# qiaozhijian/gf-orb-slam2

Measured on AMD Instinct MI355X. Metric: frames/sec ORB extract+match, 752x480 @2000 kp, higher is better.
Workload: dtype u8; 1 GPU; configs[2]: stereo 752x480 pair, 2000 features/image, extract L+R + stereo Hamming match; frame=one camera image (a stereo pair = 2 frames + 1 association), width=752, height=480, nfeatures=2000, levels=8, contexts_per_gpu=2, contexts_chained_after_stage=1, priming_steps=48, distinct_input_batches=4

## Files before the change

gf-orb-slam2_amd/csrc/gfo_api.hip:

```cpp
#include "gfo_internal.h"

#include <math.h>
#include <stdarg.h>
#include <stdio.h>
#include <stdlib.h>
#include <string.h>

static std::string g_create_err;
#include <algorithm>
#include <mutex>
#include <vector>
#include <atomic>
static std::mutex g_ctx_mu;
static std::vector<gfo_ctx*> g_ctx_live;
static std::atomic<int> g_contexts_created{0}, g_arenas_planned{0};

int gfo_fail(gfo_ctx* c, int code, const char* fmt, ...)
{
    char buf[512];
    va_list ap;
    va_start(ap, fmt);
    vsnprintf(buf, sizeof buf, fmt, ap);
    va_end(ap);
    if (c) c->err = buf;
// ... 95 lines not shown
    c->quota[n - 1] = c->prm.nfeatures - sum > 0 ? c->prm.nfeatures - sum : 0;
}

static void free_arena(gfo_ctx* c)
{
    void* ptrs[] = {c->d_geom, c->d_input, c->d_pyr, c->d_blur, c->d_cand, c->d_cand_cnt, c->d_node_of, c->d_sel,
                    c->d_sel_cnt, c->d_kp, c->d_desc, c->d_kp_cnt, c->d_flags, c->d_xofs, c->d_xcoef, c->d_yofs, c->d_band, c->d_cell_tab, c->d_qt_scratch,
                    c->d_ycoef, c->st.u_right, c->st.depth, c->st.best_dist, c->st.best_idx, c->st.nmatched, c->st.counted,
                    c->d_scale, c->d_inv_scale, c->d_kp_un, c->st_sort.sx, c->st_sort.sy, c->st_sort.soi, c->st_sort.sdesc, c->st_sort.row_start, c->st_sort.lorder, c->st_sort.lrow_start};
    for (void* p : ptrs)
        if (p) (void)hipFree(p);
    c->d_geom = nullptr; c->d_input = c->d_pyr = c->d_blur = nullptr; c->d_cand = nullptr; c->d_cand_cnt = nullptr;
    c->d_node_of = nullptr; c->d_sel = nullptr; c->d_sel_cnt = nullptr; c->d_kp = nullptr; c->d_desc = nullptr;
    c->d_kp_cnt = nullptr; c->d_flags = nullptr; c->d_xofs = nullptr; c->d_xcoef = nullptr; c->d_yofs = nullptr; c->d_band = nullptr; c->d_cell_tab = nullptr; c->d_od_tab = nullptr; c->od_pairs = 0; c->d_qt_scratch = nullptr;
    c->d_ycoef = nullptr; c->st = GfoStereoDev{}; c->d_scale = nullptr; c->d_inv_scale = nullptr; c->d_kp_un = nullptr; c->st_sort = GfoStereoSort{}; c->st_rows_cap = 0;
    c->planned = false;
    c->have_batch = c->have_pyramid = c->have_stereo = false;
    c->plan_gen++;
    if (c->graph_exec) {
        (void)hipGraphExecDestroy(c->graph_exec);
        c->graph_exec = nullptr;
    }
}

static void resize_tables(int ssize, int dsize, int* ofs, short* coef, bool clamp_x)
{
    const double inv_scale = (double)dsize / ssize;
    const double scale = 1. / inv_scale;
    for (int d = 0; d < dsize; d++) {
        float f = (float)((d + 0.5) * scale - 0.5);
        int s = (int)floorf(f);
        f -= s;
        if (clamp_x) {
            if (s < 0) { f = 0; s = 0; }
            if (s >= ssize - 1) { f = 0; s = ssize - 1; }
        }
        ofs[d] = s;
        coef[2 * d] = (short)lrintf((1.f - f) * 2048.f);
        coef[2 * d + 1] = (short)lrintf(f * 2048.f);
    }
}

#if GFO_OCV_RESIZE == 1
static void resize_tables_float(int ssize, int dsize, int* ofs, int* frac_bits)
{
    const double scale = 1. / ((double)dsize / ssize);
    for (int d = 0; d < dsize; d++) {
        float f = (float)((d + 0.5) * scale - 0.5);
        int s = (int)floorf(f);
        f -= s;
        if (s < 0) { f = 0; s = 0; }
        if (s >= ssize - 1) { f = 0; s = ssize - 1; }
        ofs[d] = s;
        memcpy(&frac_bits[d], &f, 4);
    }
}
#endif

int gfo_plan(gfo_ctx* c, int w, int h, int batch)
{
    if (c->planned && c->g.w0 == w && c->g.h0 == h && batch <= c->cap_batch) return GFO_OK;
    if (w > 4000 || h > 4000) return fail(c, GFO_ERR_INVALID, "image %dx%d exceeds the 4000-px coordinate packing", w, h);
    const int keep_batch = c->planned && c->g.w0 == w && c->g.h0 == h ? c->cap_batch : 0;
    (void)hipStreamSynchronize(c->stream);
    free_arena(c);
    batch = batch > keep_batch ? batch : keep_batch;
    if (batch < c->prm.max_batch) batch = c->prm.max_batch;
    GfoGeom& g = c->g;
    memset(&g, 0, sizeof g);
    g.nlevels = c->prm.nlevels;
    g.w0 = w;
    g.h0 = h;
    g.ini_th = c->prm.ini_th_fast;
    g.min_th = c->prm.min_th_fast;
    long long pyr_off = 0, blur_off = 0, cand_off = 0;
    int cell_base = 0, tile_base = 0, blur_b = 0, sel_off = 0, xtab = 0, ytab = 0;
    int max_cw = 8, max_ch = 8;
    for (int l = 0; l < g.nlevels; l++) {
        GfoLevel& L = g.lv[l];
        const float s = c->inv_scale[l];
        L.w = (int)lrintf((float)w * s);
        L.h = (int)lrintf((float)h * s);
        if (L.w < 1 || L.h < 1) return fail(c, GFO_ERR_INVALID, "level %d of a %dx%d image is empty", l, w, h);
        L.pitch = (int)align_up(L.w, 64);
        L.plane_off = pyr_off;
        if (l > 0) pyr_off += align_up((long long)L.pitch * L.h, 256);
        L.blur_off = blur_off;
        blur_off += align_up((long long)L.pitch * L.h, 256);
        L.max_bx = L.w - GFO_EDGE + 3;
        L.max_by = L.h - GFO_EDGE + 3;
        const float width = (float)(L.max_bx - GFO_MIN_BORDER), height = (float)(L.max_by - GFO_MIN_BORDER);
        L.cell_base = cell_base;
        if (width >= (float)GFO_CELL_W && height >= (float)GFO_CELL_W) {
            L.ncols = (int)(width / GFO_CELL_W);
            L.nrows = (int)(height / GFO_CELL_W);
            L.wcell = (int)ceilf(width / L.ncols);
            L.hcell = (int)ceilf(height / L.nrows);
            cell_base += L.ncols * L.nrows;
            max_cw = L.wcell + 6 > max_cw ? L.wcell + 6 : max_cw;
            max_ch = L.hcell + 6 > max_ch ? L.hcell + 6 : max_ch;
            L.cand_cap = L.ncols * L.nrows * ((L.wcell + 1) / 2) * ((L.hcell + 1) / 2);
        } else {
            L.ncols = L.nrows = 0;
            L.wcell = L.hcell = 1;
            L.cand_cap = 0;
        }
        L.cand_off = cand_off;
        cand_off += align_up(L.cand_cap, 64);
        L.tiles_x = (L.w + 3) / 4;
        L.tiles_y = (L.h + GFO_BLUR_STRIP - 1) / GFO_BLUR_STRIP;
        {
            int nint = (L.w - 8) / 4;
            if (nint > L.tiles_x - 1) nint = L.tiles_x - 1;
            if (nint < 0) nint = 0;
            L.tile_base = tile_base;
            tile_base += (nint * L.tiles_y + 255) / 256;
            L.blur_base_b = blur_b;
            blur_b += ((L.tiles_x - nint) * L.tiles_y + 255) / 256;
        }
        L.quota = c->quota[l];
        int nini = 1;
        if (L.max_by - GFO_MIN_BORDER > 0) nini = (int)roundf(width / height);
        if (nini < 1) nini = 1;
        L.n_ini = nini;
        L.hx = width / nini;
        L.node_cap = (L.quota > 4 * nini ? L.quota : 4 * nini) + 8;
        L.sel_off = sel_off;
        L.sel_cap = L.node_cap;
        sel_off += L.sel_cap;
        L.scale = c->scale[l];
        L.patch_size = (int)(GFO_PATCH * c->scale[l]);
        L.xtab_off = xtab;
        L.ytab_off = ytab;
        if (l > 0) {
            xtab += (int)align_up(L.w + 3, 4) + 4;
            ytab += (int)align_up(L.h + 3, 4) + 4;
        }
        if (L.node_cap > 60000) return fail(c, GFO_ERR_INVALID, "level %d takes %d of the %d features: more than 60000 nodes per level are not supported", l, L.quota, c->prm.nfeatures);
    }
    if (max_cw - 6 > 64 || max_ch - 6 > 64)
        return fail(c, GFO_ERR_INVALID, "FAST cell %dx%d exceeds the per-wave plan", max_cw - 6, max_ch - 6);
    const int xtab_n = xtab, ytab_n = ytab;
    g.total_cells = cell_base;
    g.total_tiles = tile_base;
    g.blur_total_b = blur_b;
    g.total_sel_cap = sel_off;
    g.kp_stride = (int)align_up(sel_off, 4);
    g.fast_tile_pitch = max_cw <= 45 ? 48 : (max_cw <= 61 ? 64 : 80);
    g.fast_npx_max = (int)align_up((long long)(max_cw - 6) * (max_ch - 6), 8);
    {
        const int qcap_env = getenv("GFO_FAST_QCAP") ? atoi(getenv("GFO_FAST_QCAP")) : 0;
        const int qc = qcap_env >= 264 ? (qcap_env & ~7) : GFO_FAST_QCAP;
        g.fast_q_cap = g.fast_npx_max < qc ? g.fast_npx_max : qc;
    }
    g.fast_tile_rows = max_ch;
    g.fast_smap_pitch = g.fast_tile_pitch - 4;
    g.fast_smap_rows = (int)align_up((long long)(max_ch - 6 + 2) * g.fast_smap_pitch, 16) / g.fast_smap_pitch + 1;
    g.pyr_img_stride = align_up(pyr_off, 256);
    g.blur_img_stride = align_up(blur_off, 256);
    g.cand_img_stride = align_up(cand_off, 64);
    if (g.kp_stride > 65535) return fail(c, GFO_ERR_INVALID, "more than 65535 keypoints per image are not supported");

    std::vector<int> xtabv(2 * (size_t)(xtab_n > 0 ? xtab_n : 4)), ytabv(2 * (size_t)(ytab_n > 0 ? ytab_n : 4));
    for (int l = 1; l < g.nlevels; l++) {
        const int dw = g.lv[l].w, dh = g.lv[l].h;
        std::vector<int> ofs(dw > dh ? dw : dh);
        std::vector<short> coef(2 * ofs.size());
#if GFO_OCV_RESIZE == 1
        std::vector<int> fb(ofs.size());
        resize_tables_float(g.lv[l - 1].w, dw, ofs.data(), fb.data());
        for (int d = 0; d < dw + 3 + 4; d++) {
            const int s_ = d < dw ? d : dw - 1;
            if (g.lv[l].xtab_off + d >= xtab_n) break;
            xtabv[2 * (g.lv[l].xtab_off + d)] = ofs[s_];
            xtabv[2 * (g.lv[l].xtab_off + d) + 1] = fb[s_];
        }
        resize_tables_float(g.lv[l - 1].h, dh, ofs.data(), fb.data());
        for (int d = 0; d < dh + 3 + 4; d++) {
            const int s_ = d < dh ? d : dh - 1;
            if (g.lv[l].ytab_off + d >= ytab_n) break;
            ytabv[2 * (g.lv[l].ytab_off + d)] = ofs[s_];
            ytabv[2 * (g.lv[l].ytab_off + d) + 1] = fb[s_];
        }
        (void)coef;
#else
        resize_tables(g.lv[l - 1].w, dw, ofs.data(), coef.data(), true);
        for (int d = 0; d < dw + 3 + 4; d++) {
            const int s_ = d < dw ? d : dw - 1;
            if (g.lv[l].xtab_off + d >= xtab_n) break;
            xtabv[2 * (g.lv[l].xtab_off + d)] = ofs[s_];
            xtabv[2 * (g.lv[l].xtab_off + d) + 1] = (int)((unsigned short)coef[2 * s_] | ((unsigned)(unsigned short)coef[2 * s_ + 1] << 16));
        }
        resize_tables(g.lv[l - 1].h, dh, ofs.data(), coef.data(), false);
        for (int d = 0; d < dh + 3 + 4; d++) {
            const int s_ = d < dh ? d : dh - 1;
            if (g.lv[l].ytab_off + d >= ytab_n) break;
            ytabv[2 * (g.lv[l].ytab_off + d)] = ofs[s_];
            ytabv[2 * (g.lv[l].ytab_off + d) + 1] = (int)((unsigned short)coef[2 * s_] | ((unsigned)(unsigned short)coef[2 * s_ + 1] << 16));
        }
#endif
    }
    for (int l = 1; l < g.nlevels; l++) {
        GfoLevel& L = g.lv[l];
        const int sh = g.lv[l - 1].h, R = GFO_RESIZE_ROWS;
        L.rs_fast_strips = 0;
        bool cols_ok = true;
        for (int q = 0; 4 * q < L.w && cols_ok; q++) {
            const int* e = &xtabv[2 * (size_t)(L.xtab_off + 4 * q)];
            cols_ok = e[6] + 1 - e[0] < 8;
        }
        if (!cols_ok) continue;
        for (int s_ = 0; s_ * R < L.h; s_++) {
            bool ok = true;
            for (int d = s_ * R; d < std::min(s_ * R + R, L.h) && ok; d++) {
                const int sy = ytabv[2 * (size_t)(L.ytab_off + d)];
                ok = sy >= 0 && sy + 1 < sh - 1 && (d == s_ * R || sy > ytabv[2 * (size_t)(L.ytab_off + d - 1)]);
            }
            if (!ok) break;
            L.rs_fast_strips = s_ + 1;
        }
    }
    std::vector<int> bandv;
    g.pyr_nb = 0;
    c->n_band_groups = 0;
    if (g.nlevels >= 2) {
        const int budget = (getenv("GFO_PYR_LDS_KB") ? atoi(getenv("GFO_PYR_LDS_KB")) : 24) * 1024;
        const int max_group = getenv("GFO_PYR_GROUP") ? atoi(getenv("GFO_PYR_GROUP")) : 4;
        const int nl = g.nlevels;
        auto sy_of = [&](int l, int dy) {
            const int v = ytabv[2 * (size_t)(g.lv[l].ytab_off + dy)], sh = g.lv[l - 1].h;
            return v < 0 ? 0 : (v > sh - 1 ? sh - 1 : v);
        };
        double px_own = 0.0, px_done = 0.0;
        auto plan_group = [&](int lb, int le, GfoBandGroup* out_bg, std::vector<int>* out_tab, int* lp_out, int* off_out) {
            for (int nb = 1; nb <= 64; nb++) {
                if (g.lv[le - 1].h < 2 * nb && nb > 1) break;
                std::vector<int> tab(4 * (size_t)nb * nl, 0);
                int maxrows[GFO_MAX_LEVELS] = {0};
                for (int b = 0; b < nb; b++) {
                    int c0_up = 0, c1_up = 0;
                    for (int l = le - 1; l >= lb; l--) {
                        const int hl = g.lv[l].h;
                        const int o0 = (int)((long long)b * hl / nb), o1 = (int)((long long)(b + 1) * hl / nb);
                        int c0 = o0, c1 = o1;
                        if (l < le - 1 && c1_up > c0_up) {
                            const int lo = sy_of(l + 1, c0_up);
                            int hi = sy_of(l + 1, c1_up - 1) + 1;
                            if (hi > hl - 1) hi = hl - 1;
                            c0 = lo < c0 ? lo : c0;
                            c1 = hi + 1 > c1 ? hi + 1 : c1;
                        }
                        int* t = &tab[4 * ((size_t)b * nl + l)];
                        t[0] = c0; t[1] = c1; t[2] = o0; t[3] = o1;
                        if (c1 - c0 > maxrows[l]) maxrows[l] = c1 - c0;
                        c0_up = c0;
                        c1_up = c1;
                    }
                }
                int lds = 0;
                for (int l = lb; l < le - 1; l++) lds += (int)align_up((long long)align_up(g.lv[l].w, 16) * maxrows[l], 16);
                if (getenv("GFO_DEBUG_PLAN")) fprintf(stderr, "[gfo] pyramid bands, levels %d..%d: nb %d -> %d B of LDS (budget %d)\n", lb, le - 1, nb, lds, budget);
                if (lds <= budget) {
                    out_bg->lb = lb; out_bg->le = le; out_bg->nb = nb; out_bg->lds_bytes = lds;
                    int off = 0;
                    for (int l = lb; l < le - 1; l++) {
                        lp_out[l] = (int)align_up(g.lv[l].w, 16);
                        off_out[l] = off;
                        off += (int)align_up((long long)lp_out[l] * maxrows[l], 16);
                    }
                    for (int l = lb; l < le; l++) {
                        px_own += (double)g.lv[l].w * g.lv[l].h;
                        for (int b = 0; b < nb; b++) px_done += (double)g.lv[l].w * (tab[4 * ((size_t)b * nl + l) + 1] - tab[4 * ((size_t)b * nl + l)]);
                    }
                    out_tab->swap(tab);
                    return true;
                }
            }
            return false;
        };
        bool ok = true;
        int lb = 1;
        while (lb < nl && ok) {
            int take = 0;
            GfoBandGroup bg = {0, 0, 0, 0, 0};
            std::vector<int> tab;
            for (int size = (nl - lb < max_group ? nl - lb : max_group); size >= 2 && take == 0; size--)
                if (plan_group(lb, lb + size, &bg, &tab, g.band_lp, g.band_lds_off)) take = size;
            if (take == 0) {
                bg.lb = lb; bg.le = lb + 1; bg.nb = 0; bg.lds_bytes = 0;
                take = 1;
            } else {
                bg.tab_off = (int)(bandv.size() / 4);
                bandv.insert(bandv.end(), tab.begin(), tab.end());
                if (gfo_pyramid_bands_prepare(bg.lds_bytes) != 0) {
                    (void)hipGetLastError();
                    ok = false;
                    break;
                }
            }
            if (c->n_band_groups >= GFO_MAX_LEVELS) { ok = false; break; }
            c->band_groups[c->n_band_groups++] = bg;
            if (bg.nb > 0) g.pyr_nb = g.pyr_nb == 0 || bg.nb < g.pyr_nb ? bg.nb : g.pyr_nb;
            lb += take;
        }
        if (getenv("GFO_DEBUG_PLAN") && px_own > 0) fprintf(stderr, "[gfo] pyramid bands: %d groups, computed / owned pixels = %.3f\n", c->n_band_groups, px_done / px_own);
        const double max_over = getenv("GFO_PYR_MAX_OVERHEAD") ? atof(getenv("GFO_PYR_MAX_OVERHEAD")) : 1.30;
// ... 1464 lines not shown
```

gf-orb-slam2_amd/csrc/gfo_internal.h:

```cpp
#ifndef GFO_INTERNAL_H
#define GFO_INTERNAL_H

#include <hip/hip_runtime.h>
#include <hip/hip_ext.h>
#include <stdint.h>
#include <stdlib.h>
#include <string.h>
#include <memory>
#include <string>
#include <vector>

#include "../../include/gfo.h"
#include "../../include/gfo_undistort.h"

#ifndef GFO_RESIZE_ROWS
#define GFO_RESIZE_ROWS 8
#endif

#ifndef GFO_OCV_RESIZE
#define GFO_OCV_RESIZE 0
#endif
#ifndef GFO_OCV_ATAN_FMA
#define GFO_OCV_ATAN_FMA 0
#endif
#ifndef GFO_OCV_BLUR_ROUND
#define GFO_OCV_BLUR_ROUND 0
#endif
#ifndef GFO_GAUSS_TAPS
#define GFO_GAUSS_TAPS 18, 34, 49, 55
#endif

#define GFO_EDGE 19
#define GFO_HALF_PATCH 15
#define GFO_PATCH 31
#define GFO_MIN_BORDER 16
#ifndef GFO_FAST_QCAP
#define GFO_FAST_QCAP 768
#endif
#define GFO_FAST_XOFF 1
#define GFO_CELL_W 30
#define GFO_CNT_STRIDE 32

#ifndef GFO_BLUR_STRIP
#define GFO_BLUR_STRIP 24
#endif

struct GfoLevel {
    int w, h, pitch;
    long long plane_off;
    long long blur_off;
    int ncols, nrows, wcell, hcell;
    int max_bx, max_by;
    int cell_base;
    int tiles_x, tiles_y, tile_base;
    int blur_base_b;
    int quota;
    int n_ini;
    float hx;
    int node_cap;
    long long cand_off;
    int cand_cap;
    int sel_off, sel_cap;
    float scale;
    int patch_size;
    int xtab_off, ytab_off;
    int rs_fast_strips;
};

struct GfoBandGroup {
    int lb, le, nb, lds_bytes, tab_off;
};

struct GfoGeom {
    int nlevels;
    int w0, h0;
    int total_cells;
    int total_tiles;
    int blur_total_b;
    int total_sel_cap;
    int kp_stride;
    int ini_th, min_th;
    int fast_tile_pitch, fast_tile_rows, fast_smap_pitch, fast_smap_rows;
    int fast_npx_max;
    int fast_q_cap;
    long long pyr_img_stride;
    long long blur_img_stride;
    long long cand_img_stride;
    int pyr_nb;
    int band_lds_off[GFO_MAX_LEVELS], band_lp[GFO_MAX_LEVELS];
    GfoLevel lv[GFO_MAX_LEVELS];
};

struct GfoInput {
    const uint8_t* base;
    long long pitch;
    long long img_stride;
};

struct GfoStereoDev {
    float* u_right;
    float* depth;
    int* best_dist;
    int* best_idx;
    int* nmatched;
    unsigned char* counted;
};

#define GFO_PACK_MAX 10
struct GfoPack {
    const uint4* src[GFO_PACK_MAX];
    uint4* dst[GFO_PACK_MAX];
    int n16[GFO_PACK_MAX];
    int nseg;
    int cut_pairs;
    const int* cut_cnt_dev;
    int cut_nl_host;
    GfoStereoDev cut_out;
    int cut_out_stride;
    float* h_u_right;
    float* h_depth;
    int* h_nmatched;
};

struct GfoStereoSort {
    float* sx;
    float* sy;
    unsigned* soi;
    uint8_t* sdesc;
    int* row_start;
    int* lorder;
    int* lrow_start;
};

struct GfoStereoLaunch {
    const gfo_keypoint* kl; const uint8_t* dl;
    const gfo_keypoint* kr; const uint8_t* dr;
    const int* cnt_dev; int nl_host, nr_host;
    long long pair_stride_kp;
    int npairs;
    const float* d_scale;
    gfo_stereo_params p;
    const float* min_d; const float* max_d; long long win_stride;
    GfoStereoDev out; int out_stride;
    GfoStereoSort sort; int sort_stride;
    int window;
    int nlevels;
    bool cut_in_pack;
};

struct GfoProjBuf {
    void* base = nullptr;
    int frames_cap = 0, m_cap = 0, n_cap = 0;
    int* cell_start = nullptr;
    void* cell_xy = nullptr;
    unsigned* cell_meta = nullptr;
    void* cand = nullptr;
    int* pick = nullptr;
    int* pick_dist = nullptr;
    unsigned* live = nullptr;
    int* rot_bin = nullptr;
    int* spill_off = nullptr;
    unsigned long long* spill = nullptr;
    int spill_cap = 0;
    int* tab_g = nullptr;
    int* counters = nullptr;
    int* out_mp = nullptr;
    int* out_score = nullptr;
    int* out_q = nullptr;
};

enum GfoStage {
    ST_RESIZE = 0, ST_BLUR, ST_FAST, ST_QUADTREE, ST_ORIENT_DESC, ST_STEREO_BUCKET, ST_STEREO, ST_STEREO_CUT,
    ST_PROJECT, ST_BOW, ST_UNDISTORT, ST_COUNT
};

struct GfoEngine;
struct GfoPair;

struct gfo_ctx {
    gfo_params prm{};
    uint64_t id = 0;
    int device = 0;
    hipStream_t own_stream = nullptr;
    hipStream_t stream = nullptr;
    hipStream_t side_stream = nullptr;
    hipEvent_t ev_fork = nullptr, ev_join = nullptr;
    bool zero_cnt_pending = false;
    gfo_ctx* chain_after = nullptr;
    hipEvent_t ev_pace = nullptr;
    int pace_stage = 0;
    bool pace_recorded = false;
    bool fork_blur = true;
    std::string err;
    std::string launch_err;
    bool debug_sync = false;
    int cur_stage = 0;
    std::vector<float> scale, inv_scale, sigma2, inv_sigma2;
    std::vector<int> quota;
    int umax[16]{};
    bool planned = false;
    GfoGeom g{};
    GfoGeom* d_geom = nullptr;
    int cap_batch = 0;
    uint8_t* d_input = nullptr;
    uint8_t* d_pyr = nullptr;
    uint8_t* d_blur = nullptr;
    uint32_t* d_cand = nullptr;
    int* d_cand_cnt = nullptr;
    uint16_t* d_node_of = nullptr;
    uint32_t* d_sel = nullptr;
    int* d_sel_cnt = nullptr;
    gfo_keypoint* d_kp = nullptr;
    uint8_t* d_desc = nullptr;
    int* d_kp_cnt = nullptr;
    int* d_flags = nullptr;
    int* d_xofs = nullptr;
    short* d_xcoef = nullptr;
    int* d_yofs = nullptr;
    uint8_t* d_qt_scratch = nullptr;
    size_t qt_scratch_stride = 0;
    size_t qt_lds_granted = 0;
    int* d_cell_tab = nullptr;
    int* d_od_tab = nullptr;
    int od_pairs = 0;
    int* d_band = nullptr;
    GfoBandGroup band_groups[GFO_MAX_LEVELS];
    int n_band_groups = 0, band_threads = 0;
    short* d_ycoef = nullptr;
    float* d_scale = nullptr;
    float* d_inv_scale = nullptr;
    GfoStereoDev st{};
    GfoStereoSort st_sort{};
    int st_rows_cap = 0;
    int last_nimg = 0;
    GfoInput last_in{};
    bool have_batch = false;
    bool have_pyramid = false;
// ... 192 lines not shown
```

gf-orb-slam2_amd/csrc/k_fast.hip:

```cpp
#include "gfo_internal.h"
#include <stdlib.h>

__device__ __forceinline__ void wave_sync()
{
    __builtin_amdgcn_fence(__ATOMIC_RELEASE, "wavefront");
    __builtin_amdgcn_wave_barrier();
    __builtin_amdgcn_fence(__ATOMIC_ACQUIRE, "wavefront");
}

typedef short __attribute__((ext_vector_type(2))) s16x2;
__device__ __forceinline__ unsigned pmin(unsigned a, unsigned b)
{
    return __builtin_bit_cast(unsigned, __builtin_elementwise_min(__builtin_bit_cast(s16x2, a), __builtin_bit_cast(s16x2, b)));
}
__device__ __forceinline__ unsigned pmax(unsigned a, unsigned b)
{
    return __builtin_bit_cast(unsigned, __builtin_elementwise_max(__builtin_bit_cast(s16x2, a), __builtin_bit_cast(s16x2, b)));
}
__device__ __forceinline__ unsigned rot16(unsigned a)
{
#ifdef GFO_FAST_ALIGNBIT_ROT
    return __builtin_amdgcn_alignbit(a, a, 16);
#else
    const s16x2 v = __builtin_bit_cast(s16x2, a);
    return __builtin_bit_cast(unsigned, __builtin_shufflevector(v, v, 1, 0));
#endif
}

template <int TP>
__device__ __forceinline__ int corner_score(const uint8_t* __restrict__ tl, int tq, unsigned long long& m_run)
{
    constexpr int RB = 3 * TP + 3 + GFO_FAST_XOFF;
#ifdef GFO_FAST_RING64
    struct __attribute__((packed)) row8 { unsigned lo, hi; };
    const row8 Rm3 = *reinterpret_cast<const row8*>(tl + RB - 3 * TP - 3), Rm2 = *reinterpret_cast<const row8*>(tl + RB - 2 * TP - 3),
               Rm1 = *reinterpret_cast<const row8*>(tl + RB - TP - 3), R0 = *reinterpret_cast<const row8*>(tl + RB - 3),
               Rp1 = *reinterpret_cast<const row8*>(tl + RB + TP - 3), Rp2 = *reinterpret_cast<const row8*>(tl + RB + 2 * TP - 3),
               Rp3 = *reinterpret_cast<const row8*>(tl + RB + 3 * TP - 3);
#define GFO_SEL(b0, b1) ((unsigned)(b0) | (0x0Cu << 8) | ((unsigned)(b1) << 16) | (0x0Cu << 24))
    const unsigned v2 = __builtin_amdgcn_perm(0u, R0.lo, GFO_SEL(3, 3));
    unsigned Q[8];
    Q[0] = __builtin_amdgcn_perm(Rm3.lo, Rp3.lo, GFO_SEL(3, 4 + 3));
    Q[1] = __builtin_amdgcn_perm(Rm3.lo, Rp3.hi, GFO_SEL(0, 4 + 2));
    Q[2] = __builtin_amdgcn_perm(Rm2.lo, Rp2.hi, GFO_SEL(1, 4 + 1));
    Q[3] = __builtin_amdgcn_perm(Rm1.lo, Rp1.hi, GFO_SEL(2, 4 + 0));
    Q[4] = __builtin_amdgcn_perm(R0.lo, R0.hi, GFO_SEL(2, 4 + 0));
    Q[5] = __builtin_amdgcn_perm(Rp1.lo, Rm1.hi, GFO_SEL(2, 4 + 0));
    Q[6] = __builtin_amdgcn_perm(Rp2.lo, Rm2.hi, GFO_SEL(1, 4 + 1));
    Q[7] = __builtin_amdgcn_perm(Rp3.lo, Rm3.hi, GFO_SEL(0, 4 + 2));
#undef GFO_SEL
#else
    const unsigned v = tl[RB];
    const unsigned v2 = v | (v << 16);
    const unsigned r[16] = {tl[RB + 3 * TP], tl[RB + 3 * TP + 1], tl[RB + 2 * TP + 2], tl[RB + TP + 3], tl[RB + 3], tl[RB - TP + 3], tl[RB - 2 * TP + 2], tl[RB - 3 * TP + 1],
                            tl[RB - 3 * TP], tl[RB - 3 * TP - 1], tl[RB - 2 * TP - 2], tl[RB - TP - 3], tl[RB - 3], tl[RB + TP - 3], tl[RB + 2 * TP - 2], tl[RB + 3 * TP - 1]};
    unsigned Q[8];
#pragma unroll
    for (int k = 0; k < 8; k++) Q[k] = r[k] | (r[k + 8] << 16);
#endif
    const unsigned tq2 = (unsigned)tq * 0x10001u;
    const unsigned A = pmax(pmin(Q[0], rot16(Q[0])), pmin(Q[4], rot16(Q[4])));
    const unsigned B = pmin(pmax(Q[0], rot16(Q[0])), pmax(Q[4], rot16(Q[4])));
    const int vmt = (int)(v2 - tq2), vpt = (int)(v2 + tq2);
    const bool dark = (int)A < vmt, bright = (int)B > vpt;
    const unsigned long long m_dark = __builtin_amdgcn_ballot_w64(dark), m_bright = __builtin_amdgcn_ballot_w64(bright);
    unsigned long long m_neg = ~m_dark;
    if ((m_dark & m_bright) != 0) {
        const unsigned e1 = pmin(Q[1], rot16(Q[1])), e2 = pmin(Q[2], rot16(Q[2])), e3 = pmin(Q[3], rot16(Q[3]));
        const unsigned e5 = pmin(Q[5], rot16(Q[5])), e6 = pmin(Q[6], rot16(Q[6])), e7 = pmin(Q[7], rot16(Q[7]));
        const unsigned m8 = pmax(pmax(pmax(e1, e2), pmax(e3, e5)), pmax(pmax(e6, e7), A));
        const unsigned long long m_all8 = __builtin_amdgcn_ballot_w64((int)m8 < vmt);
        m_neg |= m_bright & ~m_all8;
    }
    const bool neg = __builtin_amdgcn_inverse_ballot_w64(m_neg);
    m_run = m_dark | m_bright;
    int best = 0;
    {
        const s16x2 nsg = __builtin_bit_cast(s16x2, neg ? 0x00010001u : 0xFFFFFFFFu);
        const s16x2 sv = __builtin_bit_cast(s16x2, v2) * __builtin_bit_cast(s16x2, neg ? 0xFFFFFFFFu : 0x00010001u);
        unsigned P[8];
#pragma unroll
        for (int k = 0; k < 8; k++) P[k] = __builtin_bit_cast(unsigned, __builtin_bit_cast(s16x2, Q[k]) * nsg + sv);
        const unsigned a1 = pmin(P[1], P[2]), a3 = pmin(P[3], P[4]), a5 = pmin(P[5], P[6]), a7 = pmin(P[7], rot16(P[0]));
        const unsigned b1 = pmin(a1, a3), b3 = pmin(a3, a5), b5 = pmin(a5, a7), b7 = pmin(a7, rot16(a1));
        const unsigned c1 = pmin(b1, b5), c3 = pmin(b3, b7), c5 = pmin(b5, rot16(b1)), c7 = pmin(b7, rot16(b3));
        unsigned bst = pmin(c1, pmax(P[0], rot16(P[1])));
        bst = pmax(bst, pmin(c3, pmax(P[2], rot16(P[3]))));
        bst = pmax(bst, pmin(c5, pmax(P[4], rot16(P[5]))));
        bst = pmax(bst, pmin(c7, pmax(P[6], rot16(P[7]))));
        const int b0 = (int)(short)(bst & 0xFFFF), b1s = (int)(short)(bst >> 16);
        best = max(b0, b1s);
    }
    return best;
}

#ifndef GFO_FAST_PREFILTER
#define GFO_FAST_PREFILTER 0
#endif
#define GFO_FAST_RING_BYTES 0

template <int TP, int SP, bool XCD8>
__global__ __launch_bounds__(256) void k_fast(const GfoGeom* __restrict__ gp, GfoInput in,
                                              const uint8_t* __restrict__ pyr, uint32_t* __restrict__ cand,
                                              int* __restrict__ cand_cnt, int* __restrict__ flags, const int* __restrict__ cell_tab,
                                              int nimg
#ifdef GFO_FAST_DEBUG
                                              , int dbg_stop
#endif
                                              )
{
    extern __shared__ __attribute__((aligned(16))) uint8_t lds[];
    const GfoGeom& g = *gp;
    const int wave = __builtin_amdgcn_readfirstlane(threadIdx.x >> 6), lane = threadIdx.x & 63;
    const int img = XCD8 ? (int)(blockIdx.y * 8 + (blockIdx.x & 7)) : (int)blockIdx.y;
    if (XCD8 && img >= nimg) return;
    const int cell = (int)(XCD8 ? blockIdx.x >> 3 : blockIdx.x) * (int)(blockDim.x >> 6) + wave;
    const int tile_bytes = TP * g.fast_tile_rows, smap_bytes = (SP * g.fast_smap_rows + 15) & ~15;
#if GFO_FAST_PREFILTER
    const bool prefilter = g.fast_q_cap < g.fast_npx_max && g.fast_q_cap >= 512;
    const int q_cap = prefilter ? g.fast_q_cap - 128 : g.fast_q_cap;
#else
    const int q_cap = g.fast_q_cap;
#endif
    const bool q_capped = q_cap < g.fast_npx_max;
    const int per_wave = tile_bytes + smap_bytes + 2 * g.fast_q_cap;
    uint8_t* tile = lds + wave * per_wave;
    uint8_t* smap = tile + tile_bytes;
    unsigned short* qa = reinterpret_cast<unsigned short*>(smap + smap_bytes);
    unsigned short* qb = qa;
#if GFO_FAST_PREFILTER
    unsigned short* ring = qa + q_cap;
#endif

    if (cell >= g.total_cells) return;
    const int4 ct = reinterpret_cast<const int4*>(cell_tab)[cell];
    const int ce = __builtin_amdgcn_readfirstlane(ct.x);
    const int map_ld = __builtin_amdgcn_readfirstlane(ct.y), map_a = __builtin_amdgcn_readfirstlane(ct.z);
    const int level = ce & 15, ci = (ce >> 4) & 0xFFF, cj = ce >> 16;
    const GfoLevel& L = g.lv[level];
    const int wcell = L.wcell, hcell = L.hcell;
    const int iniX = GFO_MIN_BORDER + cj * wcell, iniY = GFO_MIN_BORDER + ci * hcell;
    const int maxX = min(iniX + wcell + 6, L.max_bx), maxY = min(iniY + hcell + 6, L.max_by);
    if (iniY >= L.max_by - 3 || iniX >= L.max_bx - 6) return;
    const int cw = maxX - iniX, ch = maxY - iniY;
    const int sw = cw - 6, sh = ch - 6;
    if (sw <= 0 || sh <= 0) return;
    constexpr int xoff = GFO_FAST_XOFF;
    struct __attribute__((packed)) seg16 { uint32_t a, b, c, d; };
    {
        int pitch;
        const uint8_t* src = gfo_level_ptr(g, in, pyr, level, img, &pitch);
        src += (long long)iniY * pitch + (iniX - xoff);
        const int spr = map_ld & 31;
        const int rps = (map_ld >> 5) & 127;
        const int lr = (lane * (map_ld >> 12)) >> 12;
        const int lc = lane - lr * spr;
        const bool ld_on = lr < rps;
        const unsigned o_last = (unsigned)((ch - 1) * pitch + 16 * lc);
        const unsigned o_first = (unsigned)(min(lr, ch - 1) * pitch + 16 * lc);
        const unsigned gstep = (unsigned)(rps * pitch);
        uint4* t128 = reinterpret_cast<uint4*>(tile) + lr * (TP >> 4) + lc;
        const int lstep = rps * (TP >> 4);
        if (2 * rps >= ch) {
            const seg16 sa = *reinterpret_cast<const seg16*>(src + o_first);
            const seg16 sb = *reinterpret_cast<const seg16*>(src + (rps + lr < ch ? o_first + gstep : o_last));
            const uint4 va = make_uint4(sa.a, sa.b, sa.c, sa.d), vb = make_uint4(sb.a, sb.b, sb.c, sb.d);
            if (ld_on && lr < ch) t128[0] = va;
            if (ld_on && rps + lr < ch) t128[lstep] = vb;
        } else {
            uint4 v[6];
#pragma unroll
            for (int k = 0; k < 6; k++) {
                if (k * rps < ch) {
                    const seg16 sk = *reinterpret_cast<const seg16*>(src + (k * rps + lr < ch ? o_first + k * gstep : o_last));
                    v[k] = make_uint4(sk.a, sk.b, sk.c, sk.d);
                }
            }
#pragma unroll
            for (int k = 0; k < 6; k++)
                if (k * rps < ch && ld_on && k * rps + lr < ch) t128[k * lstep] = v[k];
        }
        uint4* sm128 = reinterpret_cast<uint4*>(smap);
        const uint4 z4 = make_uint4(0, 0, 0, 0);
        for (int t = lane; t < ((sh + 2) * SP + 15) >> 4; t += 64) sm128[t] = z4;
    }
    wave_sync();
#ifdef GFO_FAST_DEBUG
    if (dbg_stop == 1) return;
#endif
    int total = 0, nb = 0;
    for (int round = 0; round < 2; round++) {
    const int tq = round == 0 ? g.ini_th : g.min_th;
    int na = 0;
    bool dense = false;
    nb = 0;
    auto score_queued = [&](int from) {
        const unsigned short* qr = qa + from + lane;
        for (int i0 = from; i0 < na; i0 += 64, qr += 64) {
            const int rem = na - i0;
            const unsigned long long m_in = rem >= 64 ? ~0ull : (1ull << rem) - 1ull;
            int p = 0;
            if (__builtin_amdgcn_inverse_ballot_w64(m_in)) p = *qr;
            const int py = p >> 6, px = p & 63;
            unsigned long long m_run;
            const int sc = corner_score<TP>(tile + py * TP + px, tq, m_run);
            const unsigned long long m = __builtin_amdgcn_ballot_w64(sc > tq) & m_in & m_run;
            unsigned short* qw = qb + nb;
            if (__builtin_amdgcn_inverse_ballot_w64(m)) {
                smap[(py + 1) * SP + px + 1] = (uint8_t)sc;
                if (!dense) qw[__builtin_amdgcn_mbcnt_hi((unsigned)(m >> 32), __builtin_amdgcn_mbcnt_lo((unsigned)m, 0u))] = (unsigned short)p;
            }
            nb += __popcll(m);
        }
    };
    {
        const uint32_t* t32 = reinterpret_cast<const uint32_t*>(tile);
        const int tp4 = TP >> 2;
        const int nq = map_a & 31;
        const int rpi = (map_a >> 5) & 127;
        const int lr = (lane * (map_a >> 12)) >> 12;
        const int lq = lane - lr * nq;
        const bool lane_on = lr < rpi;
        const int c0 = 4 * lq;
        const unsigned tq2 = (unsigned)tq | ((unsigned)tq << 16);
        const int nv = sw - c0;
        const unsigned tq_e = (nv > 0 ? (unsigned)tq : 0x7FFFu) | ((nv > 2 ? (unsigned)tq : 0x7FFFu) << 16);
        const unsigned tq_o = (nv > 1 ? (unsigned)tq : 0x7FFFu) | ((nv > 3 ? (unsigned)tq : 0x7FFFu) << 16);
        (void)tq2;
        int idx = (lr + 3) * tp4 + 1 + lq;
        int p0 = (lr << 6) + c0;
#if GFO_FAST_PREFILTER
        if (round == 0 && prefilter) {
            const int nv_last = sw - 4 * (nq - 1);
            const unsigned tq_full = (unsigned)tq | ((unsigned)tq << 16);
            const unsigned tq_e_last = (nv_last > 0 ? (unsigned)tq : 0x7FFFu) | ((nv_last > 2 ? (unsigned)tq : 0x7FFFu) << 16);
            const unsigned tq_o_last = (nv_last > 1 ? (unsigned)tq : 0x7FFFu) | ((nv_last > 3 ? (unsigned)tq : 0x7FFFu) << 16);
            int wr = 0, rd = 0;
            auto full_pass = [&](int cnt) {
                if (q_capped && na + 256 > q_cap) {
                    wave_sync();
                    score_queued(dense ? 0 : nb);
                    wave_sync();
                    na = dense ? 0 : nb;
                    if (!dense && nb + 256 > q_cap) {
                        dense = true;
                        na = 0;
                    }
                }
                const unsigned long long m_in = cnt >= 64 ? ~0ull : (1ull << cnt) - 1ull;
                unsigned t_e = 0, t_o = 0;
                int pd = 0;
                if (__builtin_amdgcn_inverse_ballot_w64(m_in)) {
                    pd = ring[(rd + lane) & 127];
                    const int py = pd >> 6, px = pd & 63;
                    const int di = (py + 3) * tp4 + 1 + (px >> 2);
                    const unsigned C = t32[di], Wm = t32[di - 1], Wp = t32[di + 1];
                    const unsigned U = t32[di + 3 * tp4], D = t32[di - 3 * tp4];
                    const unsigned Lw = __builtin_amdgcn_alignbyte(C, Wm, 1);
                    const unsigned Rw = __builtin_amdgcn_alignbyte(Wp, C, 3);
                    const bool last = (px >> 2) == nq - 1;
                    const unsigned te_l = last ? tq_e_last : tq_full, to_l = last ? tq_o_last : tq_full;
#pragma unroll
                    for (int h = 0; h < 2; h++) {
                        const unsigned ps = h ? 0x0C030C01u : 0x0C020C00u;
                        const s16x2 vc = __builtin_bit_cast(s16x2, __builtin_amdgcn_perm(0u, C, ps));
                        const s16x2 pu = __builtin_bit_cast(s16x2, __builtin_amdgcn_perm(0u, U, ps));
                        const s16x2 pr = __builtin_bit_cast(s16x2, __builtin_amdgcn_perm(0u, Rw, ps));
                        const s16x2 pdn = __builtin_bit_cast(s16x2, __builtin_amdgcn_perm(0u, D, ps));
                        const s16x2 pl = __builtin_bit_cast(s16x2, __builtin_amdgcn_perm(0u, Lw, ps));
                        const s16x2 dk = vc - __builtin_elementwise_max(__builtin_elementwise_min(pu, pdn), __builtin_elementwise_min(pr, pl));
                        const s16x2 br = __builtin_elementwise_min(__builtin_elementwise_max(pu, pdn), __builtin_elementwise_max(pr, pl)) - vc;
                        const unsigned t1 = __builtin_bit_cast(unsigned, __builtin_bit_cast(s16x2, h ? to_l : te_l) - __builtin_elementwise_max(dk, br));
                        if (h) t_o = t1; else t_e = t1;
                    }
                }
#pragma unroll
                for (int j = 0; j < 4; j++) {
                    const unsigned tw = (j & 1) ? t_o : t_e;
                    unsigned long long m;
                    if (j & 2) m = __builtin_amdgcn_ballot_w64((int)tw < 0);
                    else asm("v_cmp_gt_i16_e64 %0, 0, %1" : "=s"(m) : "v"(tw));
                    unsigned short* qj = qa + na;
                    if (__builtin_amdgcn_inverse_ballot_w64(m)) qj[__builtin_amdgcn_mbcnt_hi((unsigned)(m >> 32), __builtin_amdgcn_mbcnt_lo((unsigned)m, 0u))] = (unsigned short)(pd + j);
                    na += __popcll(m);
                }
                rd += cnt;
            };
            for (int y0 = 0; y0 < sh; y0 += rpi, idx += rpi * tp4, p0 += rpi << 6) {
                bool keep = false;
                if (lane_on && lr < sh - y0) {
                    const unsigned C = t32[idx], Wm = t32[idx - 1], Wp = t32[idx + 1];
                    const unsigned U = t32[idx + 3 * tp4], D = t32[idx - 3 * tp4];
                    const unsigned Lw = __builtin_amdgcn_alignbyte(C, Wm, 1);
                    const unsigned Rw = __builtin_amdgcn_alignbyte(Wp, C, 3);
                    const unsigned sv = max(__builtin_amdgcn_sad_u8(C, U, 0u), __builtin_amdgcn_sad_u8(C, D, 0u));
                    const unsigned shz = max(__builtin_amdgcn_sad_u8(C, Lw, 0u), __builtin_amdgcn_sad_u8(C, Rw, 0u));
                    keep = min(sv, shz) > (unsigned)tq;
                }
                const unsigned long long m = __builtin_amdgcn_ballot_w64(keep);
                if (__builtin_amdgcn_inverse_ballot_w64(m))
                    ring[(wr + (int)__builtin_amdgcn_mbcnt_hi((unsigned)(m >> 32), __builtin_amdgcn_mbcnt_lo((unsigned)m, 0u))) & 127] = (unsigned short)p0;
                wr += __popcll(m);
                if (wr - rd >= 64) {
                    wave_sync();
                    full_pass(64);
                }
            }
            if (wr - rd > 0) {
                wave_sync();
                full_pass(wr - rd);
            }
        } else
#endif
        for (int y0 = 0; y0 < sh; y0 += rpi, idx += rpi * tp4, p0 += rpi << 6) {
            if (q_capped && na + 256 > q_cap) {
                wave_sync();
                score_queued(dense ? 0 : nb);
                wave_sync();
                na = dense ? 0 : nb;
                if (!dense && nb + 256 > q_cap) {
                    dense = true;
                    na = 0;
                }
            }
            unsigned t_e = 0, t_o = 0;
            if (lane_on && lr < sh - y0) {
                const unsigned C = t32[idx], Wm = t32[idx - 1], Wp = t32[idx + 1];
                const unsigned U = t32[idx + 3 * tp4], D = t32[idx - 3 * tp4];
                const unsigned Lw = __builtin_amdgcn_alignbyte(C, Wm, 1);
                const unsigned Rw = __builtin_amdgcn_alignbyte(Wp, C, 3);
#pragma unroll
                for (int h = 0; h < 2; h++) {
                    const unsigned ps = h ? 0x0C030C01u : 0x0C020C00u;
                    const s16x2 vc = __builtin_bit_cast(s16x2, __builtin_amdgcn_perm(0u, C, ps));
                    const s16x2 pu = __builtin_bit_cast(s16x2, __builtin_amdgcn_perm(0u, U, ps));
                    const s16x2 pr = __builtin_bit_cast(s16x2, __builtin_amdgcn_perm(0u, Rw, ps));
                    const s16x2 pd = __builtin_bit_cast(s16x2, __builtin_amdgcn_perm(0u, D, ps));
                    const s16x2 pl = __builtin_bit_cast(s16x2, __builtin_amdgcn_perm(0u, Lw, ps));
                    const s16x2 dk = vc - __builtin_elementwise_max(__builtin_elementwise_min(pu, pd), __builtin_elementwise_min(pr, pl));
                    const s16x2 br = __builtin_elementwise_min(__builtin_elementwise_max(pu, pd), __builtin_elementwise_max(pr, pl)) - vc;
                    const unsigned t1 = __builtin_bit_cast(unsigned, __builtin_bit_cast(s16x2, h ? tq_o : tq_e) - __builtin_elementwise_max(dk, br));
                    if (h) t_o = t1; else t_e = t1;
                }
            }
#pragma unroll
            for (int j = 0; j < 4; j++) {
                const unsigned tw = (j & 1) ? t_o : t_e;
                unsigned long long m;
                if (j & 2) m = __builtin_amdgcn_ballot_w64((int)tw < 0);
                else asm("v_cmp_gt_i16_e64 %0, 0, %1" : "=s"(m) : "v"(tw));
                unsigned short* qj = qa + na;
                if (__builtin_amdgcn_inverse_ballot_w64(m)) qj[__builtin_amdgcn_mbcnt_hi((unsigned)(m >> 32), __builtin_amdgcn_mbcnt_lo((unsigned)m, 0u))] = (unsigned short)(p0 + j);
                na += __popcll(m);
            }
        }
    }
    wave_sync();
#ifdef GFO_FAST_DEBUG
    if (dbg_stop == 2) { if (na == 12345) flags[1] = 1; return; }
#endif
    score_queued(dense ? 0 : nb);
    wave_sync();
#ifdef GFO_FAST_DEBUG
    if (dbg_stop == 3) { if (nb == 12345) flags[1] = 1; return; }
    if (dbg_stop == 4 && round == 1) return;
    if (dbg_stop == 9) { if (lane == 0) { atomicAdd(&flags[1], sw * sh); atomicAdd(&flags[2], na); atomicAdd(&flags[3], nb); } }
#endif
    int n_max = 0;
    uint32_t* keyq = reinterpret_cast<uint32_t*>(tile);
    const unsigned short* qn = qb + lane;
    const int n_steps = dense ? 64 * sh : nb;
    for (int i0 = 0; i0 < n_steps; i0 += 64, qn += 64) {
        unsigned long long m_in;
        int p = 0;
        if (dense) {
            p = ((i0 >> 6) << 6) | min(lane, sw - 1);
            m_in = sw >= 64 ? ~0ull : (1ull << sw) - 1ull;
        } else {
            const int rem = nb - i0;
            m_in = rem >= 64 ? ~0ull : (1ull << rem) - 1ull;
            if (__builtin_amdgcn_inverse_ballot_w64(m_in)) p = *qn;
        }
        const int py = p >> 6, px = p & 63;
        const uint8_t* q = smap + (py + 1) * SP + px + 1;
        const int s = q[0];
        const int nmax = max(max(max(max((int)q[-1], (int)q[1]), max((int)q[-SP - 1], (int)q[-SP])),
                                 max(max((int)q[-SP + 1], (int)q[SP - 1]), max((int)q[SP], (int)q[SP + 1]))), tq);
        const unsigned long long m = __builtin_amdgcn_ballot_w64(s > nmax) & m_in;
        const int x = px + 3 + cj * wcell, y = py + 3 + ci * hcell;
        const uint32_t key = (uint32_t)x | ((uint32_t)y << 12) | ((uint32_t)(s - 1) << 24);
        uint32_t* kw = keyq + n_max;
        if (__builtin_amdgcn_inverse_ballot_w64(m)) kw[__builtin_amdgcn_mbcnt_hi((unsigned)(m >> 32), __builtin_amdgcn_mbcnt_lo((unsigned)m, 0u))] = key;
        n_max += __popcll(m);
    }
    wave_sync();
    total = n_max;
    if (total > 0) break;
    }
    if (total == 0) return;
    int base = 0;
    int* cnt = cand_cnt + (img * g.nlevels + level) * GFO_CNT_STRIDE;
    if (lane == 0) base = atomicAdd(cnt, total);
    base = __shfl(base, 0);
    if (base + total > L.cand_cap) {
        if (lane == 0) atomicOr(&flags[0], 1);
        return;
    }
    uint32_t* out = cand + (long long)img * g.cand_img_stride + L.cand_off + base;
    const uint32_t* keyq = reinterpret_cast<const uint32_t*>(tile);
    for (int i = lane; i < total; i += 64) out[i] = keyq[i];
}

void gfo_launch_fast(gfo_ctx* c, const GfoInput& in, int nimg)
{
    const GfoGeom& g = c->g;
    if (g.total_cells == 0) return;
    static const int nw_env = getenv("GFO_FAST_WAVES") ? atoi(getenv("GFO_FAST_WAVES")) : 0;
    const int nw = nw_env >= 1 && nw_env <= 4 ? nw_env : 1;
    const size_t lds = nw * (size_t)(g.fast_tile_pitch * g.fast_tile_rows + ((g.fast_smap_pitch * g.fast_smap_rows + 15) & ~15) + 2 * g.fast_q_cap);
    const int cell_blocks = (g.total_cells + nw - 1) / nw;
    static const int xcd_env = getenv("GFO_FAST_XCD") ? atoi(getenv("GFO_FAST_XCD")) : 1;
    const bool xcd8 = xcd_env && nimg >= 8;
    const dim3 grid = xcd8 ? dim3((unsigned)cell_blocks * 8u, (unsigned)(nimg + 7) / 8u) : dim3(cell_blocks, nimg);
    gfo_prof_begin(c, ST_FAST);
#ifdef GFO_FAST_DEBUG
    static const int dbg_stop = getenv("GFO_FAST_STOP") ? atoi(getenv("GFO_FAST_STOP")) : 0;
#define GFO_FAST_DBG_ARG , dbg_stop
#else
#define GFO_FAST_DBG_ARG
#endif
#define GFO_FAST_LAUNCH(TP_, SP_)                                                                                       \
    do {                                                                                                                \
        if (xcd8)                                                                                                       \
            GFO_LAUNCH(c, (k_fast<TP_, SP_, true>), grid, dim3(64 * nw), lds, c->stream, c->d_geom, in, c->d_pyr, c->d_cand, \
                               c->d_cand_cnt, c->d_flags, c->d_cell_tab, nimg GFO_FAST_DBG_ARG);                        \
        else                                                                                                            \
            GFO_LAUNCH(c, (k_fast<TP_, SP_, false>), grid, dim3(64 * nw), lds, c->stream, c->d_geom, in, c->d_pyr, c->d_cand, \
                               c->d_cand_cnt, c->d_flags, c->d_cell_tab, nimg GFO_FAST_DBG_ARG);                        \
    } while (0)
    if (g.fast_tile_pitch == 48) GFO_FAST_LAUNCH(48, 44);
    else if (g.fast_tile_pitch == 64) GFO_FAST_LAUNCH(64, 60);
    else GFO_FAST_LAUNCH(80, 76);
#undef GFO_FAST_LAUNCH
#undef GFO_FAST_DBG_ARG
    gfo_prof_end(c);
}

void gfo_kernels_fast(std::vector<const void*>& v)
{
#ifndef GFO_FAST_DEBUG
    v.push_back((const void*)k_fast<48, 44, true>); v.push_back((const void*)k_fast<48, 44, false>);
    v.push_back((const void*)k_fast<64, 60, true>); v.push_back((const void*)k_fast<64, 60, false>);
    v.push_back((const void*)k_fast<80, 76, true>); v.push_back((const void*)k_fast<80, 76, false>);
#else
    (void)v;
#endif
}
```

Measured before the change: 300,700 frames/s.

## Process runs of FAST cells per wave with optional next-tile prefetch

```diff
diff --git a/gf-orb-slam2_amd/csrc/gfo_api.hip b/gf-orb-slam2_amd/csrc/gfo_api.hip
--- a/gf-orb-slam2_amd/csrc/gfo_api.hip
+++ b/gf-orb-slam2_amd/csrc/gfo_api.hip
@@ -271,6 +271,9 @@
         const int qcap_env = getenv("GFO_FAST_QCAP") ? atoi(getenv("GFO_FAST_QCAP")) : 0;
         const int qc = qcap_env >= 264 ? (qcap_env & ~7) : GFO_FAST_QCAP;
         g.fast_q_cap = g.fast_npx_max < qc ? g.fast_npx_max : qc;
+        const int run_env = getenv("GFO_FAST_RUN") ? atoi(getenv("GFO_FAST_RUN")) : 0;
+        g.fast_run = run_env >= 1 && run_env <= 16 ? run_env : GFO_FAST_RUN;
+        if (getenv("GFO_DEBUG_PLAN")) fprintf(stderr, "[gfo] k_fast: %d cells, runs of %d cell(s) per wave, queue of %d entries\n", g.total_cells, g.fast_run, g.fast_q_cap);
     }
     g.fast_tile_rows = max_ch;
     g.fast_smap_pitch = g.fast_tile_pitch - 4;
diff --git a/gf-orb-slam2_amd/csrc/gfo_internal.h b/gf-orb-slam2_amd/csrc/gfo_internal.h
--- a/gf-orb-slam2_amd/csrc/gfo_internal.h
+++ b/gf-orb-slam2_amd/csrc/gfo_internal.h
@@ -36,6 +36,9 @@
 #define GFO_MIN_BORDER 16
 #ifndef GFO_FAST_QCAP
 #define GFO_FAST_QCAP 768
+#endif
+#ifndef GFO_FAST_RUN
+#define GFO_FAST_RUN 2
 #endif
 #define GFO_FAST_XOFF 1
 #define GFO_CELL_W 30
@@ -83,6 +86,7 @@
     int fast_tile_pitch, fast_tile_rows, fast_smap_pitch, fast_smap_rows;
     int fast_npx_max;
     int fast_q_cap;
+    int fast_run;
     long long pyr_img_stride;
     long long blur_img_stride;
     long long cand_img_stride;
diff --git a/gf-orb-slam2_amd/csrc/k_fast.hip b/gf-orb-slam2_amd/csrc/k_fast.hip
--- a/gf-orb-slam2_amd/csrc/k_fast.hip
+++ b/gf-orb-slam2_amd/csrc/k_fast.hip
@@ -97,10 +97,13 @@
 #ifndef GFO_FAST_PREFILTER
 #define GFO_FAST_PREFILTER 0
 #endif
+#ifndef GFO_FAST_EMIT_OVERLAP
+#define GFO_FAST_EMIT_OVERLAP 0
+#endif
 #define GFO_FAST_RING_BYTES 0
 
 template <int TP, int SP, bool XCD8>
-__global__ __launch_bounds__(256) void k_fast(const GfoGeom* __restrict__ gp, GfoInput in,
+__global__ __launch_bounds__(256) __attribute__((amdgpu_waves_per_eu(8, 8))) void k_fast(const GfoGeom* __restrict__ gp, GfoInput in,
                                               const uint8_t* __restrict__ pyr, uint32_t* __restrict__ cand,
                                               int* __restrict__ cand_cnt, int* __restrict__ flags, const int* __restrict__ cell_tab,
                                               int nimg
@@ -114,7 +117,9 @@
     const int wave = __builtin_amdgcn_readfirstlane(threadIdx.x >> 6), lane = threadIdx.x & 63;
     const int img = XCD8 ? (int)(blockIdx.y * 8 + (blockIdx.x & 7)) : (int)blockIdx.y;
     if (XCD8 && img >= nimg) return;
-    const int cell = (int)(XCD8 ? blockIdx.x >> 3 : blockIdx.x) * (int)(blockDim.x >> 6) + wave;
+    const int wave_idx = (int)(XCD8 ? blockIdx.x >> 3 : blockIdx.x) * (int)(blockDim.x >> 6) + wave;
+    const int run = g.fast_run;
+    const int cell_end = min((wave_idx + 1) * run, g.total_cells);
     const int tile_bytes = TP * g.fast_tile_rows, smap_bytes = (SP * g.fast_smap_rows + 15) & ~15;
 #if GFO_FAST_PREFILTER
     const bool prefilter = g.fast_q_cap < g.fast_npx_max && g.fast_q_cap >= 512;
@@ -132,28 +137,62 @@
     unsigned short* ring = qa + q_cap;
 #endif
 
-    if (cell >= g.total_cells) return;
-    const int4 ct = reinterpret_cast<const int4*>(cell_tab)[cell];
-    const int ce = __builtin_amdgcn_readfirstlane(ct.x);
-    const int map_ld = __builtin_amdgcn_readfirstlane(ct.y), map_a = __builtin_amdgcn_readfirstlane(ct.z);
-    const int level = ce & 15, ci = (ce >> 4) & 0xFFF, cj = ce >> 16;
-    const GfoLevel& L = g.lv[level];
-    const int wcell = L.wcell, hcell = L.hcell;
-    const int iniX = GFO_MIN_BORDER + cj * wcell, iniY = GFO_MIN_BORDER + ci * hcell;
-    const int maxX = min(iniX + wcell + 6, L.max_bx), maxY = min(iniY + hcell + 6, L.max_by);
-    if (iniY >= L.max_by - 3 || iniX >= L.max_bx - 6) return;
-    const int cw = maxX - iniX, ch = maxY - iniY;
-    const int sw = cw - 6, sh = ch - 6;
-    if (sw <= 0 || sh <= 0) return;
+    struct cell_geo {
+        int level, x0, y0;
+        int map_ld, map_a;
+        int cw, ch;
+        bool ok;
+    };
+    auto geo_of = [&](int cell) {
+        cell_geo G;
+        const int4 ct = reinterpret_cast<const int4*>(cell_tab)[cell];
+        const int ce = __builtin_amdgcn_readfirstlane(ct.x);
+        G.map_ld = __builtin_amdgcn_readfirstlane(ct.y);
+        G.map_a = __builtin_amdgcn_readfirstlane(ct.z);
+        G.level = ce & 15;
+        const GfoLevel& L = g.lv[G.level];
+        G.x0 = (ce >> 16) * L.wcell;
+        G.y0 = ((ce >> 4) & 0xFFF) * L.hcell;
+        const int iniX = GFO_MIN_BORDER + G.x0, iniY = GFO_MIN_BORDER + G.y0;
+        G.cw = min(iniX + L.wcell + 6, L.max_bx) - iniX;
+        G.ch = min(iniY + L.hcell + 6, L.max_by) - iniY;
+        G.ok = !(iniY >= L.max_by - 3 || iniX >= L.max_bx - 6) && G.cw > 6 && G.ch > 6;
+        return G;
+    };
     constexpr int xoff = GFO_FAST_XOFF;
     struct __attribute__((packed)) seg16 { uint32_t a, b, c, d; };
-    {
+    auto two_step = [&](const cell_geo& G) { return 2 * ((G.map_ld >> 5) & 127) >= G.ch; };
+    auto tile_issue2 = [&](const cell_geo& G, uint4& va, uint4& vb) {
         int pitch;
-        const uint8_t* src = gfo_level_ptr(g, in, pyr, level, img, &pitch);
-        src += (long long)iniY * pitch + (iniX - xoff);
-        const int spr = map_ld & 31;
-        const int rps = (map_ld >> 5) & 127;
-        const int lr = (lane * (map_ld >> 12)) >> 12;
+        const uint8_t* src = gfo_level_ptr(g, in, pyr, G.level, img, &pitch);
+        src += (long long)(GFO_MIN_BORDER + G.y0) * pitch + (GFO_MIN_BORDER + G.x0 - xoff);
+        const int spr = G.map_ld & 31, rps = (G.map_ld >> 5) & 127, ch = G.ch;
+        const int lr = (lane * (G.map_ld >> 12)) >> 12;
+        const int lc = lane - lr * spr;
+        const unsigned o_last = (unsigned)((ch - 1) * pitch + 16 * lc);
+        const unsigned o_first = (unsigned)(min(lr, ch - 1) * pitch + 16 * lc);
+        const unsigned gstep = (unsigned)(rps * pitch);
+        const seg16 sa = *reinterpret_cast<const seg16*>(src + o_first);
+        const seg16 sb = *reinterpret_cast<const seg16*>(src + (rps + lr < ch ? o_first + gstep : o_last));
+        va = make_uint4(sa.a, sa.b, sa.c, sa.d);
+        vb = make_uint4(sb.a, sb.b, sb.c, sb.d);
+    };
+    auto tile_store2 = [&](const cell_geo& G, const uint4& va, const uint4& vb) {
+        const int spr = G.map_ld & 31, rps = (G.map_ld >> 5) & 127, ch = G.ch;
+        const int lr = (lane * (G.map_ld >> 12)) >> 12;
+        const int lc = lane - lr * spr;
+        const bool ld_on = lr < rps;
+        uint4* t128 = reinterpret_cast<uint4*>(tile) + lr * (TP >> 4) + lc;
+        const int lstep = rps * (TP >> 4);
+        if (ld_on && lr < ch) t128[0] = va;
+        if (ld_on && rps + lr < ch) t128[lstep] = vb;
+    };
+    auto tile_load6 = [&](const cell_geo& G) {
+        int pitch;
+        const uint8_t* src = gfo_level_ptr(g, in, pyr, G.level, img, &pitch);
+        src += (long long)(GFO_MIN_BORDER + G.y0) * pitch + (GFO_MIN_BORDER + G.x0 - xoff);
+        const int spr = G.map_ld & 31, rps = (G.map_ld >> 5) & 127, ch = G.ch;
+        const int lr = (lane * (G.map_ld >> 12)) >> 12;
         const int lc = lane - lr * spr;
         const bool ld_on = lr < rps;
         const unsigned o_last = (unsigned)((ch - 1) * pitch + 16 * lc);
@@ -161,32 +200,49 @@
         const unsigned gstep = (unsigned)(rps * pitch);
         uint4* t128 = reinterpret_cast<uint4*>(tile) + lr * (TP >> 4) + lc;
         const int lstep = rps * (TP >> 4);
-        if (2 * rps >= ch) {
-            const seg16 sa = *reinterpret_cast<const seg16*>(src + o_first);
-            const seg16 sb = *reinterpret_cast<const seg16*>(src + (rps + lr < ch ? o_first + gstep : o_last));
-            const uint4 va = make_uint4(sa.a, sa.b, sa.c, sa.d), vb = make_uint4(sb.a, sb.b, sb.c, sb.d);
-            if (ld_on && lr < ch) t128[0] = va;
-            if (ld_on && rps + lr < ch) t128[lstep] = vb;
-        } else {
-            uint4 v[6];
-#pragma unroll
-            for (int k = 0; k < 6; k++) {
-                if (k * rps < ch) {
-                    const seg16 sk = *reinterpret_cast<const seg16*>(src + (k * rps + lr < ch ? o_first + k * gstep : o_last));
-                    v[k] = make_uint4(sk.a, sk.b, sk.c, sk.d);
-                }
-            }
-#pragma unroll
-            for (int k = 0; k < 6; k++)
-                if (k * rps < ch && ld_on && k * rps + lr < ch) t128[k * lstep] = v[k];
+        uint4 v[6];
+#pragma unroll
+        for (int k = 0; k < 6; k++) {
+            if (k * rps < ch) {
+                const seg16 sk = *reinterpret_cast<const seg16*>(src + (k * rps + lr < ch ? o_first + k * gstep : o_last));
+                v[k] = make_uint4(sk.a, sk.b, sk.c, sk.d);
+            }
         }
+#pragma unroll
+        for (int k = 0; k < 6; k++)
+            if (k * rps < ch && ld_on && k * rps + lr < ch) t128[k * lstep] = v[k];
+    };
+    cell_geo G = {};
+    uint4 pf_a = make_uint4(0, 0, 0, 0), pf_b = pf_a;
+    bool pf = false;
+    for (int cell = wave_idx * run; cell < cell_end; cell++) {
+    wave_sync();
+    if (!pf) {
+        G = geo_of(cell);
+        if (!G.ok) continue;
+    }
+    const int level = G.level;
+    const GfoLevel& L = g.lv[level];
+    const int cw = G.cw, ch = G.ch;
+    const int sw = cw - 6, sh = ch - 6;
+    const int x0 = G.x0, y0 = G.y0;
+    const int map_a = G.map_a;
+    (void)ch;
+    {
+        if (two_step(G)) {
+            if (!pf) tile_issue2(G, pf_a, pf_b);
+            tile_store2(G, pf_a, pf_b);
+        } else
+            tile_load6(G);
+        pf = false;
         uint4* sm128 = reinterpret_cast<uint4*>(smap);
         const uint4 z4 = make_uint4(0, 0, 0, 0);
         for (int t = lane; t < ((sh + 2) * SP + 15) >> 4; t += 64) sm128[t] = z4;
     }
     wave_sync();
 #ifdef GFO_FAST_DEBUG
-    if (dbg_stop == 1) return;
+    if (dbg_stop == 1) continue;
+    bool dbg_cut = false;
 #endif
     int total = 0, nb = 0;
     for (int round = 0; round < 2; round++) {
@@ -357,13 +413,13 @@
     }
     wave_sync();
 #ifdef GFO_FAST_DEBUG
-    if (dbg_stop == 2) { if (na == 12345) flags[1] = 1; return; }
+    if (dbg_stop == 2) { if (na == 12345) flags[1] = 1; dbg_cut = true; break; }
 #endif
     score_queued(dense ? 0 : nb);
     wave_sync();
 #ifdef GFO_FAST_DEBUG
-    if (dbg_stop == 3) { if (nb == 12345) flags[1] = 1; return; }
-    if (dbg_stop == 4 && round == 1) return;
+    if (dbg_stop == 3) { if (nb == 12345) flags[1] = 1; dbg_cut = true; break; }
+    if (dbg_stop == 4 && round == 1) { dbg_cut = true; break; }
     if (dbg_stop == 9) { if (lane == 0) { atomicAdd(&flags[1], sw * sh); atomicAdd(&flags[2], na); atomicAdd(&flags[3], nb); } }
 #endif
     int n_max = 0;
@@ -387,7 +443,7 @@
         const int nmax = max(max(max(max((int)q[-1], (int)q[1]), max((int)q[-SP - 1], (int)q[-SP])),
                                  max(max((int)q[-SP + 1], (int)q[SP - 1]), max((int)q[SP], (int)q[SP + 1]))), tq);
         const unsigned long long m = __builtin_amdgcn_ballot_w64(s > nmax) & m_in;
-        const int x = px + 3 + cj * wcell, y = py + 3 + ci * hcell;
+        const int x = px + 3 + x0, y = py + 3 + y0;
         const uint32_t key = (uint32_t)x | ((uint32_t)y << 12) | ((uint32_t)(s - 1) << 24);
         uint32_t* kw = keyq + n_max;
         if (__builtin_amdgcn_inverse_ballot_w64(m)) kw[__builtin_amdgcn_mbcnt_hi((unsigned)(m >> 32), __builtin_amdgcn_mbcnt_lo((unsigned)m, 0u))] = key;
@@ -397,18 +453,33 @@
     total = n_max;
     if (total > 0) break;
     }
-    if (total == 0) return;
+#ifdef GFO_FAST_DEBUG
+    if (dbg_cut) continue;
+#endif
+    if (total == 0) continue;
     int base = 0;
     int* cnt = cand_cnt + (img * g.nlevels + level) * GFO_CNT_STRIDE;
+    const int cand_cap = L.cand_cap;
+    uint32_t* out = cand + (long long)img * g.cand_img_stride + L.cand_off;
     if (lane == 0) base = atomicAdd(cnt, total);
+#if GFO_FAST_EMIT_OVERLAP
+    if (cell + 1 < cell_end) {
+        const cell_geo Gn = geo_of(cell + 1);
+        if (Gn.ok && two_step(Gn)) {
+            tile_issue2(Gn, pf_a, pf_b);
+            G = Gn;
+            pf = true;
+        }
+    }
+#endif
     base = __shfl(base, 0);
-    if (base + total > L.cand_cap) {
+    if (base + total > cand_cap) {
         if (lane == 0) atomicOr(&flags[0], 1);
-        return;
-    }
-    uint32_t* out = cand + (long long)img * g.cand_img_stride + L.cand_off + base;
+        continue;
+    }
     const uint32_t* keyq = reinterpret_cast<const uint32_t*>(tile);
-    for (int i = lane; i < total; i += 64) out[i] = keyq[i];
+    for (int i = lane; i < total; i += 64) out[base + i] = keyq[i];
+    }
 }
 
 void gfo_launch_fast(gfo_ctx* c, const GfoInput& in, int nimg)
@@ -418,7 +489,7 @@
     static const int nw_env = getenv("GFO_FAST_WAVES") ? atoi(getenv("GFO_FAST_WAVES")) : 0;
     const int nw = nw_env >= 1 && nw_env <= 4 ? nw_env : 1;
     const size_t lds = nw * (size_t)(g.fast_tile_pitch * g.fast_tile_rows + ((g.fast_smap_pitch * g.fast_smap_rows + 15) & ~15) + 2 * g.fast_q_cap);
-    const int cell_blocks = (g.total_cells + nw - 1) / nw;
+    const int cell_blocks = (g.total_cells + nw * g.fast_run - 1) / (nw * g.fast_run);
     static const int xcd_env = getenv("GFO_FAST_XCD") ? atoi(getenv("GFO_FAST_XCD")) : 1;
     const bool xcd8 = xcd_env && nimg >= 8;
     const dim3 grid = xcd8 ? dim3((unsigned)cell_blocks * 8u, (unsigned)(nimg + 7) / 8u) : dim3(cell_blocks, nimg);
```

After: 302,400 frames/s (median of 6 runs). About the same (+0.6%).
